# apache/datafusion-comet

Hardware: NVIDIA H100
Metric: rows/sec on TPC-H Q1 filter+agg (higher is better)
Workload: dtype i128

## Files before the change

datafusion-comet_b200/csrc/agg.cpp:

```cpp
#include "exec_internal.h"
#include "../../include/comet_b200.h"

#include "aot_kernels.h"
#include "ranges.h"

#include <algorithm>
#include <mutex>

namespace cb200 {

static std::mutex g_profile_mu;
static std::map<std::string, std::vector<int>> g_range_profile;

void reset_range_profiles() {
    std::lock_guard<std::mutex> lk(g_profile_mu);
    g_range_profile.clear();
}

namespace {

enum class Strategy { Undecided, Dense, Table, Stream };
enum Level { SAFE = 0, TYPE = 1, TIGHT = 2 };
constexpr int DENSE_MAX_GROUPS = 64;

constexpr int GK = CB_GID_RANGES;
struct HashFlags { int w[CB_HFLAG_WORDS]; };
int64_t round_ids(int64_t n) { return (n + GK - 1) / GK * GK; }

using ValueMasks = uint64_t[CB_MAX_COLS * 2];

uint64_t identity_word(int kind) { return kind == W_MIN ? 0x7fffffffffffffffull : kind == W_MAX ? 0x8000000000000000ull : 0; }

std::vector<int> decode_gid(int g, const std::vector<int>& cards) {
    std::vector<int> code(cards.size());
    for (int k = (int)cards.size() - 1; k >= 0; k--) { code[(size_t)k] = g % cards[(size_t)k]; g /= cards[(size_t)k]; }
    return code;
}

int grid_for(const ExecContext* ctx, int n_tiles) { return std::max(1, std::min(ctx->num_sms, n_tiles)); }

struct Kernel {
    PipelineSpec spec;
    GeneratedKernel g;
    std::shared_ptr<CompiledModule> mod;
};

void launch_named(ExecContext* ctx, const Kernel& k, const char* name, dim3 grid, dim3 block, void** args) {
    cuda_check(cudaLaunchKernel((const void*)k.mod->kernel(name), grid, block, args, 0, ctx->stream), name);
    ctx->kernel_launches++;
}

struct DenseState {
    std::vector<int> cards;
    std::vector<bool> has_null;
    DeviceBufP totals, spill, partials;
    int groups = 0;

    void regroup(ExecContext* ctx, int n_words, const std::vector<int>& word_kinds, const std::vector<int>& new_cards) {
        int new_groups = 1;
        for (int c : new_cards) new_groups *= c;
        std::vector<uint64_t> oldt((size_t)groups * n_words * 2), newt((size_t)new_groups * n_words * 2);
        cuda_check(cudaMemcpy(oldt.data(), totals->ptr, oldt.size() * 8, cudaMemcpyDeviceToHost), "regroup D2H");
        for (size_t i = 0; i < (size_t)new_groups * n_words; i++) newt[i * 2] = identity_word(word_kinds[i % (size_t)n_words]);
        for (int g = 0; g < groups; g++) {
            const std::vector<int> code = decode_gid(g, cards);
            int ng = 0, mul = 1;
            for (int k = (int)cards.size() - 1; k >= 0; k--) {
                int cd = code[(size_t)k];
                if (has_null[(size_t)k] && cd == cards[(size_t)k] - 1) cd = new_cards[(size_t)k] - 1;
                ng += cd * mul;
                mul *= new_cards[(size_t)k];
            }
            memcpy(&newt[(size_t)ng * n_words * 2], &oldt[(size_t)g * n_words * 2], (size_t)n_words * 16);
        }
        totals = host_to_device(newt.data(), newt.size() * 8, ctx, "regroup H2D");
        groups = new_groups;
    }

    void finalize(ExecContext* ctx, const Kernel& last, cb::FinParams fp, bool ungrouped, const std::vector<DType>& schema,
                  const std::vector<DictionaryP>& key_dicts, Batch& out) const {
        TraceSpan ts("agg.finalize");
        const GeneratedKernel& g = last.g;
        const int ng = groups;
        fp.totals = (cb::u64*)totals->ptr;
        fp.n_groups = ng;
        std::vector<size_t> off_v, off_n;
        size_t total_bytes = 0;
        auto take = [&](size_t n) { size_t o = total_bytes; total_bytes += (n + 15) / 16 * 16; return o; };
        for (size_t i = 0; i < g.out_cols.size(); i++) { off_v.push_back(take((size_t)ng * g.out_bytes[i])); off_n.push_back(take((size_t)ng)); }
        size_t off_present = take((size_t)ng);
        auto dbuf = std::make_shared<DeviceBuf>(total_bytes);
        for (size_t i = 0; i < g.out_cols.size(); i++) {
            fp.out[i] = (cb::u8*)dbuf->ptr + off_v[i];
            fp.outv[i] = (cb::u8*)dbuf->ptr + off_n[i];
        }
        fp.present = (cb::u8*)dbuf->ptr + off_present;
        void* args[] = {&fp};
        cuda_check(cudaLaunchKernel((const void*)last.mod->kernel(g.finalize_entry), dim3((ng + 127) / 128), dim3(128), args, 0, ctx->stream), "finalize launch");
        ctx->kernel_launches++;
        std::vector<uint8_t> hbuf(total_bytes);
        cuda_check(cudaMemcpyAsync(hbuf.data(), dbuf->ptr, total_bytes, cudaMemcpyDeviceToHost, ctx->stream), "agg results D2H"); ctx->d2h_bytes += (int64_t)(total_bytes);
        ctx->check_device_errors();
        const uint8_t* pres = hbuf.data() + off_present;
        std::vector<int> rows;
        for (int gi = 0; gi < ng; gi++) if (ungrouped || pres[(size_t)gi]) rows.push_back(gi);
        out.n_rows = (int64_t)rows.size();
// ... 166 lines not shown

struct KeyTable {
    DeviceBufP hkeys;
    int64_t hcap = 0;

    void ensure(ExecContext* ctx, const Kernel& k, IdRows& rows, int64_t incoming, int64_t remaining, int64_t rows_scanned, bool merging) {
        cudaStream_t st = ctx->stream;
        rows.ensure_flags(ctx);
        HashFlags hf;
        int64_t cnt[GK];
        const int64_t cur = rows.read_flags(ctx, hf, cnt);
        const int64_t need = cur + incoming;
        if (need + 2 >= INT32_MAX) throw ExecError(16, "", "more than 2^31 groups in one partition; lower spark.comet.b200.chunkRows");
        bool relocated = false;
        if (need > rows.max_groups) {
            int64_t nm = std::max<int64_t>(need, rows.max_groups + rows.max_groups / 4);
            if (remaining > 0 && rows_scanned == 0 && merging) {
                nm = std::max(nm, need + remaining);
            }
            if (remaining > 0 && rows_scanned > 0 && cur > 0) {
                const double ratio = std::min(1.0, 1.3 * (double)cur / (double)rows_scanned);
                const int64_t est = cur + incoming + (int64_t)(ratio * (double)remaining);
                nm = std::max(nm, std::min<int64_t>(est, cur + incoming + remaining));
            }
            if (nm + 2 + GK >= INT32_MAX) nm = INT32_MAX - 3 - GK;
            relocated = cur > 0;
            rows.grow(ctx, k, cnt, round_ids(nm), true);
        }
        int64_t cap = std::max<int64_t>(hcap, 1 << 16);
        while (cap < 2 * std::max(need, rows.max_groups)) cap <<= 1;
        if (cap != hcap || relocated) {
            auto nkeys = cap != hcap ? std::make_shared<DeviceBuf>((size_t)cap * 16) : hkeys;
            cuda_check(cudaMemsetAsync(nkeys->ptr, 0xff, (size_t)cap * 16, st), "memset key slots");
            if (cur > 0) {
                const cb::u64* kog = (const cb::u64*)rows.hkey_of_gid->ptr;
                int rr = (int)(rows.max_groups / GK);
                const int* ctr = (const int*)rows.hflags->ptr + CB_HFLAG_CTR;
                cb::u64* kp = (cb::u64*)nkeys->ptr;
                cb::u32 mask = (cb::u32)(cap - 1);
                void* a2[] = {&kog, &rr, &ctr, &kp, &mask};
                launch_named(ctx, k, "cb_hash_rehash", dim3((unsigned)((rows.max_groups + 255) / 256)), dim3(256), a2);
                cuda_check(cudaStreamSynchronize(st), "rehash");
            }
            hkeys = nkeys; hcap = cap;
        }
    }
};

struct StreamState {
    double ratio = 1.0;
    DeviceBufP reserved_snap;

    void ensure_rows(ExecContext* ctx, const Kernel& k, IdRows& rows, const int64_t cnt[GK], int64_t want_groups) {
        rows.ensure_flags(ctx);
        if (rows.htotals && want_groups <= rows.max_groups) return;
        rows.grow(ctx, k, cnt, round_ids(std::max<int64_t>(want_groups, rows.max_groups + rows.max_groups / 2)), false);
    }
    void snapshot_reserved(ExecContext* ctx, const IdRows& rows, int n_words, bool restore) {
        const size_t bytes = (size_t)2 * n_words * 16;
        if (!reserved_snap || reserved_snap->bytes < bytes) reserved_snap = std::make_shared<DeviceBuf>(bytes);
        cb::u64* tail = (cb::u64*)rows.htotals->ptr + (size_t)rows.max_groups * n_words * 2;
        if (restore) cuda_check(cudaMemcpyAsync(tail, reserved_snap->ptr, bytes, cudaMemcpyDeviceToDevice, ctx->stream), "restore reserved groups");
        else cuda_check(cudaMemcpyAsync(reserved_snap->ptr, tail, bytes, cudaMemcpyDeviceToDevice, ctx->stream), "snapshot reserved groups");
    }
};

struct AggNode : FusedBase {
    std::vector<ExprP> keys;
    std::vector<AggExpr> aggs;
    std::vector<std::vector<int>> state_cols;
    AggMode mode = AggMode::Partial;
    bool reads_rows = true;
    bool all_partial = true;
    std::vector<bool> is_state_col;
    bool ungrouped = false;
    bool emitted = false;
    std::vector<Batch> outq;
    size_t outq_pos = 0;
    std::vector<int> assume_bits;

    std::vector<bool> key_has_null;
    std::vector<bool> col_nullable;
    std::vector<DictionaryP> key_dicts;
    struct DevDict { StringDictDev d; std::vector<DeviceBufP> bufs; int host_known = 0; };
    std::vector<std::shared_ptr<DevDict>> dev_dicts;

    int n_words = 0, key_words = 1;
    std::vector<int> word_kinds, role_words;
    Kernel last;
    bool have_totals() const { return last.mod != nullptr; }

    Strategy strategy = Strategy::Undecided;
    DenseState dense;
    KeyTable table;
    IdRows rows;

    std::vector<int> observed_bits;
    int64_t rows_scanned = 0;
    std::string profile_key;
    DeviceBufP vmask;
    StreamState stream;

    int assume_for(int child_col, Level lv) const {
        const DType& t = child->schema[(size_t)child_col];
        if (!t.is_decimal() || lv == SAFE || !reads_rows || is_state_col[(size_t)child_col]) return 0;
        int k = r_bitlen(r_prec_max(t.precision));
        if ((size_t)child_col < assume_bits.size() && assume_bits[(size_t)child_col] > 0) k = std::min(k, assume_bits[(size_t)child_col]);
        if (lv == TIGHT && !observed_bits.empty() && observed_bits[(size_t)child_col] >= 0) k = std::min(k, observed_bits[(size_t)child_col] + 2);
        return std::min(k, 126);
    }

    PipelineSpec make_spec(const Batch* b, Strategy st, int n_groups, Level lv = TYPE) const {
        const bool hash = st == Strategy::Table || st == Strategy::Stream;
        PipelineSpec s;
        s.cols = stage_cols(b);
        for (auto& c : s.cols) {
            c.assume_bits = assume_for(c.src_index, lv);
            c.layout_nullable = b && col_nullable[(size_t)c.src_index];
        }
        s.predicates = to_slots(predicates, slot_of);
        s.sink = SinkKind::Agg;
        s.mode = mode;
        s.ungrouped = ungrouped;
        s.hash = hash;
        s.keys = to_slots(keys, slot_of);
        for (size_t k = 0; k < keys.size(); k++) s.key_nullable.push_back(b ? key_has_null[k] : false);
        for (auto& a : aggs) {
            AggExpr c = a;
            if (a.mode == AggMode::Partial) {
                c.children = to_slots(a.children, slot_of);
                if (a.filter) c.filter = to_slots({a.filter}, slot_of)[0];
            }
            s.aggs.push_back(c);
        }
        for (auto& sc : state_cols) {
            std::vector<int> v;
            for (int ci : sc) v.push_back(slot_of.at(ci));
            s.state_slots.push_back(v);
        }
        if (hash) {
            s.threads = ctx->hash_threads;
            s.tile = 2 * ctx->hash_threads;
            s.stream = st == Strategy::Stream;
        }
        GeneratedKernel probe = generate_pipeline(s);
        size_t acc = (!ungrouped && !hash) ? (size_t)std::max(n_groups, 1) * probe.n_words * s.threads * 8 : 0;
        while (acc + 2 * (size_t)probe.stage_bytes + 1024 > SMEM_BUDGET && s.threads > 32) {
            s.threads /= 2;
            acc /= 2;
        }
        if (acc + 2 * (size_t)probe.stage_bytes + 1024 > SMEM_BUDGET)
            throw Unsupported(hash ? "too many state / input columns to stage in shared memory for the hash aggregate kernel"
                                   : "too many groups x aggregates for the thread-private accumulators of the dense path");
        s.stages = (int)std::max<size_t>(2, std::min<size_t>(6, (SMEM_BUDGET - 1024 - acc) / (size_t)probe.stage_bytes));
        return s;
    }

    std::vector<PipelineSpec> build_specs() const override {
        bool hash = false;
        for (auto& k : keys) if (!k->type.is_string() && k->type.id != TypeId::Bool) hash = true;
        std::vector<PipelineSpec> out{make_spec(nullptr, hash ? Strategy::Table : Strategy::Dense, ungrouped ? 1 : 6)};
        if (hash && mode == AggMode::Partial && all_partial) out.push_back(make_spec(nullptr, Strategy::Stream, 6));
        return out;
    }

    Kernel compile(const PipelineSpec& spec) {
        Kernel k{spec, generate_pipeline(spec), nullptr};
        k.mod = jit_get(k.g, true);
        if (have_totals() && k.g.key_words != key_words) throw ExecError(15, "", "internal: group key packing changed between launches");
        if (have_totals() && (k.g.n_words != n_words || k.g.word_kinds != word_kinds || k.g.role_words != role_words)) widen(k);
        n_words = k.g.n_words;
        word_kinds = k.g.word_kinds;
        role_words = k.g.role_words;
        key_words = k.g.key_words;
        return k;
    }

    void widen(const Kernel& k) {
        GeneratedKernel from;
        from.n_words = n_words;
        from.word_kinds = word_kinds;
        from.role_words = role_words;
        const std::vector<int> map = widen_word_map(from, k.g);
        if (map.empty()) throw ExecError(15, "", "internal: accumulator layout changed between launches");
        const bool is_dense = strategy == Strategy::Dense;
        DeviceBufP& t = is_dense ? dense.totals : rows.htotals;
        const size_t n_rows = is_dense ? (size_t)dense.groups : (size_t)rows.max_groups + 2;
        auto nt = std::make_shared<DeviceBuf>(n_rows * (size_t)k.g.n_words * 16);
        for (int w = 0; w < k.g.n_words; w++)
            cuda_check(cudaMemcpy2DAsync((char*)nt->ptr + (size_t)w * 16, (size_t)k.g.n_words * 16, (const char*)t->ptr + (size_t)map[(size_t)w] * 16,
                                         (size_t)n_words * 16, 16, n_rows, cudaMemcpyDeviceToDevice, ctx->stream), "widen totals");
        cuda_check(cudaStreamSynchronize(ctx->stream), "widen totals");
        t = nt;
    }

    void clear_vmask() {
        if (!vmask) vmask = std::make_shared<DeviceBuf>(CB_MAX_COLS * 16);
        cuda_check(cudaMemsetAsync(vmask->ptr, 0, CB_MAX_COLS * 16, ctx->stream), "memset vmask");
    }
    void copy_vmask(ValueMasks& masks) {
        cuda_check(cudaMemcpyAsync(masks, vmask->ptr, sizeof(ValueMasks), cudaMemcpyDeviceToHost, ctx->stream), "read value masks"); ctx->d2h_bytes += (int64_t)(sizeof(ValueMasks));
    }
    static std::vector<int> mask_bits(const PipelineSpec& spec, const ValueMasks& masks) {
        std::vector<int> seen(spec.cols.size(), -1);
        for (size_t i = 0; i < spec.cols.size(); i++) {
            if (!spec.cols[i].type.is_decimal()) continue;
            uint64_t lo = masks[2 * i], hi = masks[2 * i + 1];
            seen[i] = hi ? 64 + r_bitlen(hi) : r_bitlen(lo);
        }
        return seen;
    }
    void observe(const std::vector<int>& seen) {
        for (size_t i = 0; i < seen.size(); i++)
            if (seen[i] >= 0) observed_bits[(size_t)used_cols[i]] = std::max(observed_bits[(size_t)used_cols[i]], seen[i]);
    }

    int prepare_key(Batch& b, size_t k) {
        int ci = keys[k]->index;
        Column& c = b.cols[ci];
        if (c.type.id == TypeId::Bool) return 2;
        if (!c.type.is_string()) return -1;
        if (c.is_dict) {
            key_dicts[k] = c.dict;
            return (int)c.dict->values().size();
        }
        if (!dev_dicts[k]) {
            auto dd = std::make_shared<DevDict>();
            const int64_t cap = 1 << 16;
            const int max_codes = 4096;
            const int64_t bytes_cap = 1 << 20;
            auto alloc = [&](size_t n) { auto bfr = std::make_shared<DeviceBuf>(n); cuda_check(cudaMemsetAsync(bfr->ptr, 0, bfr->bytes, ctx->stream), "memset dict"); dd->bufs.push_back(bfr); return bfr->ptr; };
            dd->d.tags = (unsigned long long*)alloc((size_t)cap * 8);
            dd->d.slot_code = (int*)alloc((size_t)cap * 4);
            dd->d.capacity = cap;
            dd->d.n_codes = (int*)alloc(64);
            dd->d.bytes_used = (unsigned long long*)((char*)dd->d.n_codes + 16);
            dd->d.err = (int*)((char*)dd->d.n_codes + 32);
            dd->d.max_codes = max_codes;
            dd->d.code_off = (long long*)alloc((size_t)max_codes * 8);
            dd->d.code_len = (int*)alloc((size_t)max_codes * 4);
            dd->d.bytes = (unsigned char*)alloc((size_t)bytes_cap);
            dd->d.bytes_cap = bytes_cap;
            dev_dicts[k] = dd;
            key_dicts[k] = std::make_shared<Dictionary>();
        }
        DevDict& dd = *dev_dicts[k];
        if (!c.offsets || !c.chars) throw Unsupported("string key column without offsets/chars buffers");
        auto row_slot = std::make_shared<DeviceBuf>((size_t)b.n_rows * 4);
        auto codes = std::make_shared<DeviceBuf>((size_t)b.n_rows * 4);
        launch_dict_encode(dd.d, (const int*)c.offsets->ptr, (const unsigned char*)c.chars->ptr, c.validity ? (const unsigned char*)c.validity->ptr : nullptr,
                           b.n_rows, (int*)row_slot->ptr, (int*)codes->ptr, ctx->stream);
        ctx->kernel_launches += 2;
        int hdr[12];
        cuda_check(cudaMemcpyAsync(hdr, dd.d.n_codes, sizeof(hdr), cudaMemcpyDeviceToHost, ctx->stream), "dict header");
        cuda_check(cudaStreamSynchronize(ctx->stream), "dict encode");
        int n_codes = hdr[0], derr = hdr[8];
        if (derr & CB_DICT_FULL) throw Unsupported("plain Utf8 group key with more distinct values than the device dictionary holds (dictionary-encode the column)");
        if (derr & CB_DICT_COLLISION) throw ExecError(14, "", "64-bit hash collision between distinct group key strings");
        if (n_codes > dd.host_known) {
            std::vector<long long> off((size_t)n_codes);
            std::vector<int> len((size_t)n_codes);
            cuda_check(cudaMemcpy(off.data(), dd.d.code_off, (size_t)n_codes * 8, cudaMemcpyDeviceToHost), "dict offsets");
            cuda_check(cudaMemcpy(len.data(), dd.d.code_len, (size_t)n_codes * 4, cudaMemcpyDeviceToHost), "dict lengths");
            for (int i = dd.host_known; i < n_codes; i++) {
                std::string s((size_t)len[(size_t)i], '\0');
                if (len[(size_t)i]) cuda_check(cudaMemcpy(&s[0], dd.d.bytes + off[(size_t)i], (size_t)len[(size_t)i], cudaMemcpyDeviceToHost), "dict bytes");
                key_dicts[k]->append(s);
            }
            dd.host_known = n_codes;
        }
        c.data = codes;
        c.phys = Phys::I32;
        c.is_dict = true;
        c.dict = key_dicts[k];
        return n_codes;
    }

    void consume(Batch& b) {
        for (int ci : used_cols) if (b.cols[(size_t)ci].validity) col_nullable[(size_t)ci] = true;
        std::vector<int> nc(keys.size());
        std::vector<bool> hn(keys.size());
        for (size_t k = 0; k < keys.size(); k++) {
            int card = prepare_key(b, k);
            const Column& c = b.cols[keys[k]->index];
            hn[k] = key_has_null[k] || c.validity != nullptr;
            nc[k] = card < 0 ? -1 : std::max(card, 1) + (hn[k] ? 1 : 0);
            if (!dense.cards.empty() && nc[k] >= 0) nc[k] = std::max(nc[k], dense.cards[k]);
        }
        bool densifiable = true;
        for (int c : nc) if (c < 0) densifiable = false;
        int n_groups = 1;
        if (densifiable) for (int c : nc) { n_groups *= c; if (n_groups > 1 << 20) break; }
        const bool needs_hash = !ungrouped && (!densifiable || n_groups > DENSE_MAX_GROUPS);
        key_has_null = hn;
        if (observed_bits.empty()) observed_bits.assign(child->schema.size(), -1);
        if (strategy == Strategy::Undecided || (strategy == Strategy::Dense && needs_hash)) {
            if (strategy == Strategy::Dense) {
                leave_dense();
                ctx->agg_strategies |= CB200_AGG_MIGRATED;
            }
            strategy = !needs_hash ? Strategy::Dense : sample_stream(b) ? Strategy::Stream : Strategy::Table;
            ctx->agg_strategies |= strategy == Strategy::Dense ? CB200_AGG_DENSE : strategy == Strategy::Stream ? CB200_AGG_STREAM : CB200_AGG_TABLE;
        }
        if (strategy == Strategy::Dense) consume_dense(b, nc, n_groups);
        else if (strategy == Strategy::Table) consume_table(b);
        else consume_stream(b);
    }

    void consume_dense(Batch& b, const std::vector<int>& nc, int n_groups) {
        if (have_totals() && nc != dense.cards) {
            if (n_words == 0) throw ExecError(15, "", "internal: regroup before layout");
            dense.regroup(ctx, n_words, word_kinds, nc);
        }
        dense.cards = nc;
        dense.has_null = key_has_null;
        const int64_t SAMPLE = 1 << 20;
        bool have_obs = false;
        for (int ci : used_cols) if (child->schema[(size_t)ci].is_decimal() && observed_bits[(size_t)ci] >= 0) have_obs = true;
        if (reads_rows && !have_obs && b.n_rows > 2 * SAMPLE) {
            profile_key = pipeline_signature(make_spec(&b, Strategy::Dense, n_groups, SAFE));
            std::lock_guard<std::mutex> lk(g_profile_mu);
            auto it = g_range_profile.find(profile_key);
            if (it != g_range_profile.end() && it->second.size() == observed_bits.size()) {
                observed_bits = it->second;
                for (int ci : used_cols) if (child->schema[(size_t)ci].is_decimal() && observed_bits[(size_t)ci] >= 0) have_obs = true;
            }
        }
        if (!reads_rows) {
            run_range(b, 0, b.n_rows, n_groups, SAFE);
        } else if (!have_obs && b.n_rows > 2 * SAMPLE) {
            run_range(b, 0, SAMPLE, n_groups, TYPE);
            run_range(b, SAMPLE, b.n_rows, n_groups, TIGHT);
        } else {
            run_range(b, 0, b.n_rows, n_groups, have_obs ? TIGHT : TYPE);
        }
        if (!profile_key.empty()) {
            std::lock_guard<std::mutex> lk(g_profile_mu);
            if (g_range_profile.size() > 256) g_range_profile.clear();
            g_range_profile[profile_key] = observed_bits;
        }
    }

    void leave_dense() {
        if (mode == AggMode::Final) throw Unsupported("group cardinality grew past the dense path mid-stream in a Final aggregate");
        if (have_totals()) {
            Batch early;
            dense.finalize(ctx, last, certified_params(), ungrouped, schema, key_dicts, early);
            if (early.n_rows > 0) outq.push_back(std::move(early));
        }
        last = Kernel();
        dense = DenseState();
        n_words = 0; word_kinds.clear(); role_words.clear(); rows_scanned = 0;
    }

    void run_range(Batch& b, int64_t row0, int64_t row1, int n_groups, Level lv) {
        TraceSpan tsr("agg.run_range");
        while (true) {
            Kernel k;
            {
                TraceSpan ts("agg.codegen+jit");
                k = compile(make_spec(&b, Strategy::Dense, n_groups, lv));
            }
            const int64_t max_rows = (int64_t)ctx->num_sms * k.g.threads * (1ll << CB_RPT_LOG2) / 1024 * 1024;
            int64_t r0 = row0;
            while (r0 < row1 && launch_one(b, r0, std::min(row1, r0 + max_rows), n_groups, k, lv)) r0 += max_rows;
            if (r0 >= row1) return;
            if (lv == SAFE) throw ExecError(15, "", "internal: value-mask validation failed without assumptions");
            lv = lv == TIGHT ? TYPE : SAFE;
            row0 = r0;
        }
    }

    bool launch_one(Batch& b, int64_t r0, int64_t r1, int n_groups, const Kernel& k, Level lv) {
        cudaStream_t st = ctx->stream;
        size_t tot_bytes = (size_t)n_groups * n_words * 16;
        if (!have_totals()) {
            dense.totals = std::make_shared<DeviceBuf>(tot_bytes);
            dense.groups = n_groups;
        }
        if (!dense.spill || dense.spill->bytes < tot_bytes) {
            dense.spill = std::make_shared<DeviceBuf>(tot_bytes);
            cuda_check(cudaMemsetAsync(dense.spill->ptr, 0, dense.spill->bytes, st), "memset spill");
        }
        clear_vmask();
        cb::PipeParams p;
        fill_inputs(p, b, k.g.tile, r0, r1);
        bind_str_masks(p, k.spec, b);
        int grid = grid_for(ctx, p.n_tiles);
        size_t part_bytes = (size_t)grid * tot_bytes;
        if (!dense.partials || dense.partials->bytes < part_bytes) dense.partials = std::make_shared<DeviceBuf>(part_bytes);
        p.n_groups = n_groups;
        for (size_t i = 0; i < dense.cards.size() && i < CB_MAX_KEYS; i++) p.key_card[i] = dense.cards[i];
        p.partials = (cb::u8*)dense.partials->ptr;
        p.spill = (cb::u64*)dense.spill->ptr;
        p.vmask = (cb::u64*)vmask->ptr;
        launch(k.mod->kernel(k.g.entry), dim3(grid), dim3(k.g.threads + 32), k.g.dyn_smem(n_groups), &p);
        ctx->pipeline_rows += r1 - r0;
        ValueMasks masks;
        copy_vmask(masks);
        const int errs = ctx->take_device_errors();
        const std::vector<int> seen = mask_bits(k.spec, masks);
        bool ok = true;
        for (size_t i = 0; i < seen.size(); i++)
            if (k.spec.cols[i].assume_bits > 0 && seen[i] > k.spec.cols[i].assume_bits) ok = false;
        observe(seen);
        if (!ok) {
            cuda_check(cudaMemsetAsync(dense.spill->ptr, 0, dense.spill->bytes, st), "memset spill");
            ctx->agg_range_reruns++;
            return false;
        }
        ctx->raise_device_errors(errs);
        ctx->agg_range_levels |= lv == TIGHT ? CB200_RANGE_TIGHT : lv == TYPE ? CB200_RANGE_TYPE : CB200_RANGE_SAFE;
        rows_scanned += r1 - r0;
        cb::FinParams fp;
        memset(&fp, 0, sizeof(fp));
        fp.partials = (const cb::u64*)dense.partials->ptr;
        fp.spill = (cb::u64*)dense.spill->ptr;
        fp.totals = (cb::u64*)dense.totals->ptr;
        fp.n_ctas = grid;
        fp.n_groups = n_groups;
        fp.first = have_totals() ? 0 : 1;
        fp.err = ctx->d_err;
        int total_words = n_groups * n_words;
        void* args[] = {&fp};
        cuda_check(cudaLaunchKernel((const void*)k.mod->kernel("cb_fold"), dim3((total_words + 127) / 128), dim3(128), args, 0, st), "fold launch");
        ctx->kernel_launches++;
        last = k;
        return true;
    }

    void launch_id_rows(Batch& b, int64_t r0, int64_t r1, const Kernel& k, bool with_table) {
        clear_vmask();
        cb::PipeParams p;
        fill_inputs(p, b, k.g.tile, r0, r1);
        bind_str_masks(p, k.spec, b);
        p.hkeys = with_table ? (cb::u64*)table.hkeys->ptr : nullptr;
        p.hkey_of_gid = (cb::u64*)rows.hkey_of_gid->ptr;
        p.htotals = (cb::u64*)rows.htotals->ptr;
        p.hmask = with_table ? (cb::u32)(table.hcap - 1) : 0;
        p.max_groups = (cb::i32)rows.max_groups;
        p.hflags = (cb::i32*)rows.hflags->ptr;
        p.vmask = (cb::u64*)vmask->ptr;
        p.n_groups = 2;
        launch(k.mod->kernel(k.g.entry), dim3(grid_for(ctx, p.n_tiles)), dim3(k.g.threads + 32), k.g.dyn_smem(0), &p);
    }

    void consume_table(Batch& b) {
        const Kernel k = compile(make_spec(&b, Strategy::Table, 2, SAFE));
        {
            TraceSpan ts("hash.ensure_table");
            table.ensure(ctx, k, rows, b.n_rows, child->rows_hint(), rows_scanned, mode != AggMode::Partial || !all_partial);
        }
        launch_id_rows(b, 0, b.n_rows, k, true);
        ctx->pipeline_rows += b.n_rows;
        ValueMasks masks;
        int flags[8];
        copy_vmask(masks);
        cuda_check(cudaMemcpyAsync(flags, rows.hflags->ptr, sizeof(flags), cudaMemcpyDeviceToHost, ctx->stream), "read hash flags"); ctx->d2h_bytes += (int64_t)(sizeof(flags));
        ctx->check_device_errors();
        if (flags[0] & CB_HF_FULL) throw ExecError(15, "", "internal: hash table full");
        if (flags[0] & CB_HF_WIDE_KEY) throw Unsupported("decimal(p > 18) group key whose value does not fit 64 bits");
        observe(mask_bits(k.spec, masks));
        rows_scanned += b.n_rows;
        last = k;
    }

    int64_t stream_launch(Batch& b, int64_t r0, int64_t r1, const Kernel& k, HashFlags& hf, int64_t cnt[GK]) {
        launch_id_rows(b, r0, r1, k, false);
        ValueMasks masks;
        copy_vmask(masks);
        ctx->check_device_errors();
        const int64_t total = rows.read_flags(ctx, hf, cnt);
        if (hf.w[0] & CB_HF_WIDE_KEY) throw Unsupported("decimal(p > 18) group key whose value does not fit 64 bits");
        if (!(hf.w[0] & CB_HF_FULL)) observe(mask_bits(k.spec, masks));
        return total;
    }
    bool sample_stream(Batch& b) {
        if (mode != AggMode::Partial || !all_partial || ctx->stream_agg_min_rows < 0) return false;
        if (b.n_rows + std::max<int64_t>(child->rows_hint(), 0) < ctx->stream_agg_min_rows || b.n_rows == 0) return false;
        const Kernel k = compile(make_spec(&b, Strategy::Stream, 2, SAFE));
        const int64_t sample = std::min<int64_t>(b.n_rows, 1 << 20);
        HashFlags hf;
        int64_t cnt[GK] = {0};
        stream.ensure_rows(ctx, k, rows, cnt, 2 * sample + 4096);
        const int64_t runs = stream_launch(b, 0, sample, k, hf, cnt);
        stream.ratio = (hf.w[0] & CB_HF_FULL) ? 1.0 : (double)runs / (double)sample;
        memset(&hf, 0, sizeof(hf));
        rows.write_flags(ctx, hf);
        IdRows::init_totals(ctx, k, (cb::u64*)rows.htotals->ptr, rows.max_groups, 2);
        if (stream.ratio <= ctx->stream_agg_max_ratio) return true;
        rows = IdRows();
        n_words = 0; word_kinds.clear(); role_words.clear();
        return false;
    }
    void consume_stream(Batch& b) {
        const Kernel k = compile(make_spec(&b, Strategy::Stream, 2, SAFE));
        HashFlags before, hf;
        int64_t cnt0[GK], cnt[GK];
        const int64_t cur = rows.read_flags(ctx, before, cnt0);
        const int64_t remaining = std::max<int64_t>(child->rows_hint(), 0);
        int64_t want = cur + std::min<int64_t>(b.n_rows, (int64_t)(1.25 * stream.ratio * (double)b.n_rows) + 65536);
        if (!rows.htotals || want > rows.max_groups) want += std::min<int64_t>(remaining, (int64_t)(1.25 * stream.ratio * (double)remaining));
        int64_t handed_out;
        while (true) {
            {
                TraceSpan ts("stream.ensure_rows");
                stream.ensure_rows(ctx, k, rows, cnt0, want);
            }
            stream.snapshot_reserved(ctx, rows, n_words, false);
            handed_out = stream_launch(b, 0, b.n_rows, k, hf, cnt);
            if (!(hf.w[0] & CB_HF_FULL)) break;
            ctx->agg_stream_reruns++;
            stream.snapshot_reserved(ctx, rows, n_words, true);
            for (int r = 0; r < GK; r++) before.w[CB_HFLAG_CTR + r] = (int)cnt0[r];
            rows.write_flags(ctx, before);
            want = cur + b.n_rows + GK;
        }
        ctx->pipeline_rows += b.n_rows;
        if (b.n_rows > 0) stream.ratio = std::max(stream.ratio, (double)(handed_out - cur) / (double)b.n_rows);
        rows_scanned += b.n_rows;
        last = k;
    }

    u128r certificate(size_t ai) const {
        const AggExpr& a = aggs[ai];
        if (!(a.kind == AggKind::Sum || a.kind == AggKind::Avg) || !a.datatype.is_decimal()) return 0;
        std::vector<u128r> bounds(child->schema.size(), RSAT);
        for (size_t c = 0; c < bounds.size(); c++)
            if (child->schema[c].is_decimal() && !observed_bits.empty())
                bounds[c] = observed_bits[c] < 0 ? 0 : (observed_bits[c] >= 127 ? RSAT : (u128r)1 << observed_bits[c]);
        if (a.mode == AggMode::Partial) return expr_maxabs(*a.children[0], bounds);
        return bounds[(size_t)state_cols[ai][0]];
    }
    cb::FinParams certified_params() const {
        cb::FinParams fp;
        memset(&fp, 0, sizeof(fp));
        fp.err = ctx->d_err;
        for (size_t ai = 0; ai < aggs.size() && ai < CB_MAX_OUT; ai++) {
            const u128r b = certificate(ai);
            fp.cert_b[ai][0] = b >= RSAT ? ~0ull : (uint64_t)b;
            fp.cert_b[ai][1] = b >= RSAT ? ~0ull : (uint64_t)(b >> 64);
            const bool direct = aggs[ai].mode != AggMode::Partial || aggs[ai].children[0]->kind == ExprKind::Bound;
            if (b < RSAT && b != 0 && direct) fp.cert_b[ai][1] |= 1ull << 63;
        }
        return fp;
    }

    bool next(Batch& out) override {
        if (!emitted) aggregate_input();
        if (outq_pos >= outq.size()) return false;
        out = std::move(outq[outq_pos++]);
        return true;
    }
    void aggregate_input() {
        if (keys.size() > CB_MAX_KEYS) throw Unsupported("more than 4 group keys");
        key_has_null.assign(keys.size(), false);
        col_nullable.assign(child->schema.size(), false);
        key_dicts.assign(keys.size(), nullptr);
        dev_dicts.assign(keys.size(), nullptr);
        Batch in;
        while (child->next(in)) {
            if (in.n_rows == 0) continue;
            consume(in);
            ctx->check_device_errors();
        }
        emitted = true;
        if (!have_totals()) {
            if (!ungrouped) return;
            last = compile(make_spec(nullptr, Strategy::Dense, 1));
            std::vector<uint64_t> id((size_t)n_words * 2, 0);
            for (int w = 0; w < n_words; w++) id[(size_t)w * 2] = identity_word(word_kinds[(size_t)w]);
            dense.totals = std::make_shared<DeviceBuf>(id.size() * 8);
            cuda_check(cudaMemcpyAsync(dense.totals->ptr, id.data(), id.size() * 8, cudaMemcpyHostToDevice, ctx->stream), "identity totals");
            cuda_check(cudaStreamSynchronize(ctx->stream), "identity totals sync");
            dense.groups = 1;
        }
        Batch result;
        if (strategy == Strategy::Table || strategy == Strategy::Stream) rows.finalize(ctx, last, certified_params(), key_dicts, result);
        else dense.finalize(ctx, last, certified_params(), ungrouped, schema, key_dicts, result);
        outq.push_back(std::move(result));
    }
};

}

ExecNodeP make_agg_node(const OperatorP& agg_op, const ExecNodeP& src, const std::vector<ExprP>& preds, const std::vector<ExprP>& cols, ExecContext* ctx,
                        const std::vector<int>& assume_bits) {
    auto n = std::make_shared<AggNode>();
    n->ctx = ctx;
    n->child = src;
    n->schema = agg_op->schema;
    n->predicates = preds;
    n->mode = agg_op->mode;
    n->ungrouped = agg_op->grouping.empty();
    n->assume_bits = assume_bits;
    std::vector<ExprP> roots = preds;
    for (auto& gexp : agg_op->grouping) {
        ExprP k = substitute(gexp, cols);
        if (k->kind != ExprKind::Bound) throw Unsupported("computed group keys (only plain column keys are fused)");
        n->keys.push_back(k);
        roots.push_back(k);
    }
    n->is_state_col.assign(src->schema.size(), false);
    n->reads_rows = agg_op->mode == AggMode::Partial;
    for (auto& a : agg_op->aggs) {
        AggExpr c = a;
        std::vector<int> sc;
        if (a.mode == AggMode::Partial) {
            n->reads_rows = true;
            for (auto& ch : c.children) { ch = substitute(ch, cols); roots.push_back(ch); }
            if (c.filter) { c.filter = substitute(c.filter, cols); roots.push_back(c.filter); }
        } else {
            n->all_partial = false;
            for (size_t k = 0; k < agg_state_types(a).size(); k++) {
                ExprP e = cols.at((size_t)a.state_at + k);
                if (e->kind != ExprKind::Bound) throw Unsupported("final aggregate over computed state columns");
                sc.push_back(e->index);
                n->is_state_col[(size_t)e->index] = true;
                roots.push_back(e);
            }
        }
        n->state_cols.push_back(sc);
        n->aggs.push_back(c);
    }
    n->assign_slots(roots);
    if (n->used_cols.empty()) {
        int best = -1, best_w = 1 << 30;
        for (size_t c = 0; c < src->schema.size(); c++) {
            const DType& t = src->schema[c];
            if (t.is_string()) continue;
            int w = std::max(1, phys_bytes(phys_of(t)));
            if (w < best_w) { best = (int)c; best_w = w; }
        }
        if (best < 0) throw Unsupported("COUNT(*) over a child with only string columns");
        n->used_cols.push_back(best);
        n->slot_of[best] = 0;
    }
    return n;
}

}
```

datafusion-comet_b200/csrc/exec.cpp:

```cpp
#include "exec_internal.h"

#include <cstdlib>
#include <ctime>
#include <mutex>

namespace cb200 {

enum { ERR_I128_OVERFLOW = 0, ERR_ANSI_OVERFLOW = 1, ERR_ORDER_DEPENDENT = 2, ERR_DIVIDE_BY_ZERO = 3, ERR_ARROW_DIVIDE_BY_ZERO = 4, ERR_DICT_CODE = 5,
       ERR_WIDE_MINMAX = 6 };

bool trace_on() {
    static int on = -1;
    if (on < 0) { const char* e = getenv("CB200_TRACE"); on = (e && *e && *e != '0') ? 1 : 0; }
    return on == 1;
}
double now_ms() {
    struct timespec ts;
    clock_gettime(CLOCK_MONOTONIC, &ts);
    return ts.tv_sec * 1e3 + ts.tv_nsec * 1e-6;
}
TraceSpan::TraceSpan(const char* n) : name(n), t0(trace_on() ? now_ms() : 0) {}
TraceSpan::~TraceSpan() {
    if (trace_on()) { static const double tz = now_ms(); const double t1 = now_ms(); fprintf(stderr, "[cb200 trace] %-28s %8.3f ms   (ends at +%.3f ms)\n", name, t1 - t0, t1 - tz); }
}
// ... 326 lines not shown
        return cudaMemcpyAsync(dst, src, n, cudaMemcpyHostToDevice, ctx->stream);
    }

    void upload(std::vector<ArrowArray>& arrs, int64_t total, Batch& out) {
        TraceSpan ts("source.upload");
        out.n_rows = total;
        out.cols.clear();
        out.cols.resize(schema.size());
        cudaStream_t st = ctx->stream;
        for (size_t c = 0; c < schema.size(); c++) {
            Column& col = out.cols[c];
            col.type = schema[c];
            bool any_nulls = false;
            for (auto& a : arrs) {
                ArrowArray* ch = a.children[c];
                if (ch->null_count != 0 && ch->buffers[0]) any_nulls = true;
            }
            if (any_nulls) {
                col.validity = std::make_shared<DeviceBuf>((size_t)(total + 7) / 8 + 8);
                cuda_check(cudaMemsetAsync(col.validity->ptr, 0, col.validity->bytes, st), "memset validity");
            }
            std::vector<DeviceBufP> temps;
            if (col_is_dict[c]) {
                col.is_dict = true;
                col.dict = dicts[c];
                int w = dict_index_width[c];
                bool need_remap = false;
                std::vector<std::vector<int32_t>> remaps;
                for (auto& a : arrs) {
                    remaps.push_back(unify_dict(c, a.children[c]->dictionary));
                    if (!remaps.back().empty()) need_remap = true;
                }
                if (!need_remap) {
                    col.phys = w == 1 ? Phys::I8 : w == 2 ? Phys::I16 : Phys::I32;
                    col.data = std::make_shared<DeviceBuf>((size_t)total * w);
                } else {
                    col.phys = Phys::I32;
                    col.data = std::make_shared<DeviceBuf>((size_t)total * 4);
                }
                int64_t row = 0;
                for (size_t k = 0; k < arrs.size(); k++) {
                    ArrowArray* ch = arrs[k].children[c];
                    const char* src = (const char*)ch->buffers[1] + ch->offset * w;
                    if (!need_remap) {
                        cuda_check(h2d((char*)col.data->ptr + row * w, src, (size_t)ch->length * w), "H2D dict codes");
                    } else {
                        auto tmp = std::make_shared<DeviceBuf>((size_t)ch->length * w);
                        temps.push_back(tmp);
                        cuda_check(h2d(tmp->ptr, src, (size_t)ch->length * w), "H2D dict codes");
                        std::vector<int32_t> table = remaps[k];
                        if (table.empty()) { table.resize((size_t)ch->dictionary->length); for (size_t i = 0; i < table.size(); i++) table[i] = (int32_t)i; }
                        DeviceBufP dt = host_to_device(table.data(), table.size() * 4, ctx, "H2D remap table");
                        ctx->h2d_bytes += (int64_t)(table.size() * 4);
                        temps.push_back(dt);
                        launch_remap_codes(tmp->ptr, w, ch->length, (const int*)dt->ptr, (int)table.size(), (int*)col.data->ptr + row, st);
                    }
                    row += ch->length;
                }
            } else if (schema[c].is_string()) {
                int64_t total_chars = 0;
                for (auto& a : arrs) {
                    ArrowArray* ch = a.children[c];
                    const int32_t* off = (const int32_t*)ch->buffers[1] + ch->offset;
                    total_chars += off[ch->length] - off[0];
                }
                if (total_chars > INT32_MAX) throw Unsupported("more than 2 GiB of string data in one chunk");
                col.chars = std::make_shared<DeviceBuf>((size_t)total_chars + 16);
                std::vector<int32_t> offs((size_t)total + 1);
                int64_t row = 0;
                int32_t base = 0;
                for (auto& a : arrs) {
                    ArrowArray* ch = a.children[c];
                    const int32_t* off = (const int32_t*)ch->buffers[1] + ch->offset;
                    for (int64_t i = 0; i < ch->length; i++) offs[(size_t)(row + i)] = base + (off[i] - off[0]);
                    int32_t nchars = off[ch->length] - off[0];
                    if (nchars) cuda_check(h2d((char*)col.chars->ptr + base, (const char*)ch->buffers[2] + off[0], (size_t)nchars), "H2D chars");
                    base += nchars;
                    row += ch->length;
                }
                offs[(size_t)total] = base;
                col.offsets = host_to_device(offs.data(), offs.size() * 4, ctx, "H2D offsets");
                ctx->h2d_bytes += (int64_t)(offs.size() * 4);
                col.phys = Phys::I32;
            } else {
                col.phys = phys_of(schema[c]);
                int w = schema[c].arrow_width();
                if (w == 0) {
                    col.data = std::make_shared<DeviceBuf>((size_t)(total + 7) / 8 + 8);
                    cuda_check(cudaMemsetAsync(col.data->ptr, 0, col.data->bytes, st), "memset bool");
                    int64_t row = 0;
                    for (auto& a : arrs) {
                        ArrowArray* ch = a.children[c];
                        append_bits((uint32_t*)col.data->ptr, row, (const uint8_t*)ch->buffers[1], ch->offset, ch->length, temps);
                        row += ch->length;
                    }
                } else {
                    col.data = std::make_shared<DeviceBuf>((size_t)total * w);
                    int64_t row = 0;
                    for (auto& a : arrs) {
                        ArrowArray* ch = a.children[c];
                        cuda_check(h2d((char*)col.data->ptr + row * w, (const char*)ch->buffers[1] + ch->offset * w, (size_t)ch->length * w), "H2D column");
                        row += ch->length;
                    }
                }
            }
            if (any_nulls) {
                int64_t row = 0, nulls = 0;
                for (auto& a : arrs) {
                    ArrowArray* ch = a.children[c];
                    bool has = ch->null_count != 0 && ch->buffers[0];
                    append_bits((uint32_t*)col.validity->ptr, row, has ? (const uint8_t*)ch->buffers[0] : nullptr, ch->offset, ch->length, temps);
                    nulls += has ? (ch->null_count < 0 ? 1 : ch->null_count) : 0;
                    row += ch->length;
                }
                col.null_count = nulls;
            }
            if (!temps.empty()) cuda_check(cudaStreamSynchronize(st), "temp buffers");
        }
    }

    void append_bits(uint32_t* dst, int64_t row, const uint8_t* src, int64_t src_off, int64_t n, std::vector<DeviceBufP>& temps) {
        if (n <= 0) return;
        if (src && (row & 7) == 0 && (src_off & 7) == 0 && ((n & 7) == 0)) {
            cuda_check(h2d((char*)dst + (row >> 3), src + (src_off >> 3), (size_t)(n >> 3)), "H2D bitmap");
            return;
        }
        const uint8_t* dsrc = nullptr;
        int64_t doff = 0;
        if (src) {
            int64_t b0 = src_off >> 3, b1 = (src_off + n + 7) >> 3;
            auto tmp = std::make_shared<DeviceBuf>((size_t)(b1 - b0) + 8);
            temps.push_back(tmp);
            cuda_check(h2d(tmp->ptr, src + b0, (size_t)(b1 - b0)), "H2D bitmap");
            dsrc = (const uint8_t*)tmp->ptr;
            doff = src_off & 7;
        }
        launch_bitmap_append(dst, row, dsrc, doff, n, ctx->stream);
    }
};

struct TableSource : ExecNode {
    std::shared_ptr<DeviceTable> table;
    ExecContext* ctx = nullptr;
    bool done = false;
    TableSource(std::shared_ptr<DeviceTable> t, const std::vector<DType>& fields, ExecContext* c) : table(std::move(t)), ctx(c) {
        schema = fields;
        if (table->cols.size() != fields.size()) throw PlanError("bound device table has " + std::to_string(table->cols.size()) + " columns, scan declares " + std::to_string(fields.size()));
    }
    int64_t pos = 0;
    bool packed = false;
    int64_t rows_hint() const override { return table->n_rows - pos; }
    bool next(Batch& out) override {
        if (done) return false;
        if (table->needs_packing && !packed) {
            for (auto& c : table->cols) {
                if (c.valid_bytes && !c.validity) c.validity = bytes_to_bitmap(c.valid_bytes, table->n_rows, ctx);
                if (c.bool_bytes && !c.data) c.data = bytes_to_bitmap(c.bool_bytes, table->n_rows, ctx);
            }
            packed = true;
        }
        const int64_t chunk = std::max<int64_t>(1024, ctx->chunk_rows / 1024 * 1024);
        const int64_t r0 = pos, r1 = std::min(table->n_rows, pos + chunk);
        pos = r1;
        if (pos >= table->n_rows) done = true;
        out.n_rows = r1 - r0;
        out.cols = table->cols;
// ... 433 lines not shown
```

datafusion-comet_b200/csrc/exec.h:

```cpp
#pragma once
#include "arrow_abi.h"
#include "codegen.h"
#include "jit.h"
#include "plan.h"

#include <cuda_runtime.h>
#include <climits>
#include <memory>
#include <string>
#include <unordered_map>
#include <vector>

namespace cb200 {

struct ExecError : std::runtime_error {
    int code;
    std::string error_class;
    ExecError(int c, const std::string& cls, const std::string& msg) : std::runtime_error(msg), code(c), error_class(cls) {}
};

void cuda_check(cudaError_t e, const char* what);

struct TraceSpan {
    const char* name;
    double t0;
    explicit TraceSpan(const char* n);
    ~TraceSpan();
};
bool trace_on();
double now_ms();
void set_alloc_stream(cudaStream_t s);
size_t release_cached_device_memory();
void reset_range_profiles();

struct DeviceBuf {
    void* ptr = nullptr;
    size_t bytes = 0;
    bool owned = true;
    cudaStream_t stream = nullptr;
    std::shared_ptr<void> owner;
    DeviceBuf() {}
    DeviceBuf(size_t n);
    DeviceBuf(void* p, size_t n) : ptr(p), bytes(n), owned(false) {}
    ~DeviceBuf();
    DeviceBuf(const DeviceBuf&) = delete;
    DeviceBuf& operator=(const DeviceBuf&) = delete;
};
using DeviceBufP = std::shared_ptr<DeviceBuf>;

class Dictionary {
  public:
    const std::vector<std::string>& values() const { return values_; }
    int32_t intern(std::string v) {
        auto it = index_.find(v);
        if (it != index_.end()) return it->second;
        if (values_.size() >= (size_t)INT32_MAX) throw Unsupported("more than 2^31 distinct strings in one dictionary");
        const int32_t code = (int32_t)values_.size();
        index_.emplace(v, code);
        values_.push_back(std::move(v));
        return code;
    }
    void append(std::string v) {
        index_.emplace(v, (int32_t)values_.size());
        values_.push_back(std::move(v));
    }
    int32_t find(const std::string& v) const {
        auto it = index_.find(v);
        return it == index_.end() ? -1 : it->second;
    }

  private:
    std::vector<std::string> values_;
    std::unordered_map<std::string, int32_t> index_;
};
using DictionaryP = std::shared_ptr<Dictionary>;

struct Column {
    DType type;
    Phys phys = Phys::I32;
    bool is_dict = false;
    DictionaryP dict;
    DeviceBufP data, validity;
    DeviceBufP offsets, chars;
    DeviceBufP valid_bytes;
    DeviceBufP bool_bytes;
    int64_t null_count = 0;
    bool on_host = false;
    std::vector<uint8_t> h_data;
    std::vector<uint8_t> h_valid;
    std::vector<int32_t> h_offsets;
};

struct Batch {
    int64_t n_rows = 0;
    std::vector<Column> cols;
};

struct ExecContext {
    int device = 0;
    cudaStream_t stream = nullptr;
    int num_sms = 132;
    int64_t chunk_rows = 1ll << 26;
    int hash_threads = 512;
    int64_t stream_agg_min_rows = 4 << 20;
    double stream_agg_max_ratio = 0.5;
    int batch_size = 8192;
    int* d_err = nullptr;
    int* h_err = nullptr;
    int64_t kernel_launches = 0;
    cudaEvent_t ev0 = nullptr, ev1 = nullptr;
    bool ev_pending = false;
    double pipeline_ms = 0;
    int64_t pipeline_launches = 0;
    int64_t pipeline_rows = 0;
    int64_t h2d_bytes = 0, d2h_bytes = 0;
    int64_t scan_pruned_row_groups = 0, scan_pruned_rows = 0;
    int64_t scan_pruned_pages = 0, scan_page_pruned_rows = 0;
    int64_t agg_strategies = 0;
    int64_t agg_range_levels = 0;
    int64_t agg_range_reruns = 0;
    int64_t sort_rows = 0, sort_passes = 0, sort_pass_rows = 0;
    int64_t sort_select_rows = 0;
    int64_t join_build_rows = 0, join_probe_rows = 0, join_out_rows = 0;
    int64_t join_cond_pairs = 0;
    double partition_ids_ms = 0, partition_place_ms = 0, partition_gather_ms = 0;
    int64_t agg_table_grows = 0;
    int64_t agg_stream_reruns = 0;
    std::vector<int64_t> partition_starts;
    void check_device_errors() { raise_device_errors(take_device_errors()); }
    int take_device_errors();
    void raise_device_errors(int e);
    void collect_timing();
};

struct ExecNode {
    std::vector<DType> schema;
    virtual ~ExecNode() {}
    virtual bool next(Batch& out) = 0;
    virtual std::vector<std::shared_ptr<ExecNode>> children() const { return {}; }
    virtual std::vector<PipelineSpec> build_specs() const { return {}; }
    virtual void push_filters(const std::vector<ExprP>&) {}
    virtual int64_t rows_hint() const { return -1; }
};
using ExecNodeP = std::shared_ptr<ExecNode>;

struct DeviceTable {
    int64_t n_rows = 0;
    std::vector<Column> cols;
    bool needs_packing = false;
};

struct PlanInputs {
    std::vector<ArrowArrayStream*> streams;
    std::vector<std::shared_ptr<DeviceTable>> tables;
};
ExecNodeP build_exec(const OperatorP& op, ExecContext* ctx, PlanInputs* inputs);

ExecNodeP make_native_scan(const OperatorP& op, ExecContext* ctx);

bool to_arrow_layout(Batch& b, ExecContext* ctx);
void export_batch(Batch& b, ExecContext* ctx, ArrowArray* out_arrays, ArrowSchema* out_schemas, int n_cols, int64_t row0, int64_t n_rows);

void register_memory_file(const std::string& name, const uint8_t* p, size_t n);
std::string describe_parquet(const std::string& path);

std::vector<GeneratedKernel> plan_kernels_for_build(const OperatorP& op, const std::vector<int>& assume_bits = {});

}
```

Measured before the change: 38.35 billion.

## Batch dense-agg range launches with a single mask readback and intern small string keys on host

Dense aggregation no longer launches, syncs and reads back value masks once per row range. It now enqueues every range kernel with its own partials, spill and mask slots, does one D2H copy and one sync, then validates and folds each range. Small plain-Utf8 key columns are interned on the host and only the codes are uploaded, and device dictionary codes are remapped to a shared host dictionary. The cost is more device memory for per-range partials, and wasted work when a range fails validation and later ranges must rerun.

```diff
diff --git a/datafusion-comet_b200/csrc/agg.cpp b/datafusion-comet_b200/csrc/agg.cpp
--- a/datafusion-comet_b200/csrc/agg.cpp
+++ b/datafusion-comet_b200/csrc/agg.cpp
@@ -22,6 +22,9 @@
 enum class Strategy { Undecided, Dense, Table, Stream };
 enum Level { SAFE = 0, TYPE = 1, TIGHT = 2 };
 constexpr int DENSE_MAX_GROUPS = 64;
+constexpr int KEY_DICT_MAX_CODES = 4096;
+constexpr int64_t KEY_DICT_MAX_BYTES = 1 << 20;
+const char* const KEY_DICT_FULL = "plain Utf8 group key with more distinct values than the device dictionary holds (dictionary-encode the column)";
 
 constexpr int GK = CB_GID_RANGES;
 struct HashFlags { int w[CB_HFLAG_WORDS]; };
@@ -354,8 +357,10 @@
     std::vector<bool> key_has_null;
     std::vector<bool> col_nullable;
     std::vector<DictionaryP> key_dicts;
-    struct DevDict { StringDictDev d; std::vector<DeviceBufP> bufs; int host_known = 0; };
+    struct DevDict { StringDictDev d; std::vector<DeviceBufP> bufs; int host_known = 0; std::vector<int32_t> to_key; };
     std::vector<std::shared_ptr<DevDict>> dev_dicts;
+    std::vector<int64_t> key_dict_bytes;
+    std::vector<std::vector<int32_t>> host_codes;
 
     int n_words = 0, key_words = 1;
     std::vector<int> word_kinds, role_words;
@@ -372,6 +377,11 @@
     std::string profile_key;
     DeviceBufP vmask;
     StreamState stream;
+    DeviceBufP range_slots;
+    std::vector<std::pair<cudaEvent_t, cudaEvent_t>> range_events;
+    ~AggNode() override {
+        for (auto& e : range_events) { cudaEventDestroy(e.first); if (e.second) cudaEventDestroy(e.second); }
+    }
 
     int assume_for(int child_col, Level lv) const {
         const DType& t = child->schema[(size_t)child_col];
@@ -496,11 +506,13 @@
             key_dicts[k] = c.dict;
             return (int)c.dict->values().size();
         }
+        if (!key_dicts[k]) key_dicts[k] = std::make_shared<Dictionary>();
+        if (!c.h_offsets.empty()) return intern_on_host(c, b.n_rows, k);
         if (!dev_dicts[k]) {
             auto dd = std::make_shared<DevDict>();
             const int64_t cap = 1 << 16;
-            const int max_codes = 4096;
-            const int64_t bytes_cap = 1 << 20;
+            const int max_codes = KEY_DICT_MAX_CODES;
+            const int64_t bytes_cap = KEY_DICT_MAX_BYTES;
             auto alloc = [&](size_t n) { auto bfr = std::make_shared<DeviceBuf>(n); cuda_check(cudaMemsetAsync(bfr->ptr, 0, bfr->bytes, ctx->stream), "memset dict"); dd->bufs.push_back(bfr); return bfr->ptr; };
             dd->d.tags = (unsigned long long*)alloc((size_t)cap * 8);
             dd->d.slot_code = (int*)alloc((size_t)cap * 4);
@@ -514,7 +526,6 @@
             dd->d.bytes = (unsigned char*)alloc((size_t)bytes_cap);
             dd->d.bytes_cap = bytes_cap;
             dev_dicts[k] = dd;
-            key_dicts[k] = std::make_shared<Dictionary>();
         }
         DevDict& dd = *dev_dicts[k];
         if (!c.offsets || !c.chars) throw Unsupported("string key column without offsets/chars buffers");
@@ -527,7 +538,7 @@
         cuda_check(cudaMemcpyAsync(hdr, dd.d.n_codes, sizeof(hdr), cudaMemcpyDeviceToHost, ctx->stream), "dict header");
         cuda_check(cudaStreamSynchronize(ctx->stream), "dict encode");
         int n_codes = hdr[0], derr = hdr[8];
-        if (derr & CB_DICT_FULL) throw Unsupported("plain Utf8 group key with more distinct values than the device dictionary holds (dictionary-encode the column)");
+        if (derr & CB_DICT_FULL) throw Unsupported(KEY_DICT_FULL);
         if (derr & CB_DICT_COLLISION) throw ExecError(14, "", "64-bit hash collision between distinct group key strings");
         if (n_codes > dd.host_known) {
             std::vector<long long> off((size_t)n_codes);
@@ -537,15 +548,50 @@
             for (int i = dd.host_known; i < n_codes; i++) {
                 std::string s((size_t)len[(size_t)i], '\0');
                 if (len[(size_t)i]) cuda_check(cudaMemcpy(&s[0], dd.d.bytes + off[(size_t)i], (size_t)len[(size_t)i], cudaMemcpyDeviceToHost), "dict bytes");
-                key_dicts[k]->append(s);
+                dd.to_key.push_back(intern_key(k, std::move(s)));
             }
             dd.host_known = n_codes;
+        }
+        bool identity = true;
+        for (size_t i = 0; i < dd.to_key.size(); i++) identity &= dd.to_key[i] == (int32_t)i;
+        if (!identity) {
+            DeviceBufP table = host_to_device(dd.to_key.data(), dd.to_key.size() * 4, ctx, "H2D key recode table");
+            launch_remap_codes(codes->ptr, 4, b.n_rows, (const int*)table->ptr, (int)dd.to_key.size(), (int*)codes->ptr, ctx->stream);
+            ctx->kernel_launches++;
+            cuda_check(cudaStreamSynchronize(ctx->stream), "key recode");
         }
         c.data = codes;
         c.phys = Phys::I32;
         c.is_dict = true;
         c.dict = key_dicts[k];
-        return n_codes;
+        return (int)key_dicts[k]->values().size();
+    }
+
+    int32_t intern_key(size_t k, std::string v) {
+        Dictionary& d = *key_dicts[k];
+        const size_t before = d.values().size(), len = v.size();
+        const int32_t code = d.intern(std::move(v));
+        if (d.values().size() > before) {
+            key_dict_bytes[k] += (int64_t)len;
+            if (d.values().size() > (size_t)KEY_DICT_MAX_CODES || key_dict_bytes[k] > KEY_DICT_MAX_BYTES) throw Unsupported(KEY_DICT_FULL);
+        }
+        return code;
+    }
+    int intern_on_host(Column& c, int64_t n_rows, size_t k) {
+        std::vector<int32_t>& codes = host_codes[k];
+        codes.assign((size_t)n_rows, 0);
+        const char* chars = (const char*)c.h_data.data();
+        for (int64_t r = 0; r < n_rows; r++) {
+            if (!c.h_valid.empty() && !c.h_valid[(size_t)r]) continue;
+            codes[(size_t)r] = intern_key(k, std::string(chars + c.h_offsets[(size_t)r], (size_t)(c.h_offsets[(size_t)r + 1] - c.h_offsets[(size_t)r])));
+        }
+        c.data = std::make_shared<DeviceBuf>((size_t)n_rows * 4);
+        cuda_check(cudaMemcpyAsync(c.data->ptr, codes.data(), codes.size() * 4, cudaMemcpyHostToDevice, ctx->stream), "H2D key codes");
+        ctx->h2d_bytes += (int64_t)(codes.size() * 4);
+        c.phys = Phys::I32;
+        c.is_dict = true;
+        c.dict = key_dicts[k];
+        return (int)key_dicts[k]->values().size();
     }
 
     void consume(Batch& b) {
@@ -634,8 +680,7 @@
                 k = compile(make_spec(&b, Strategy::Dense, n_groups, lv));
             }
             const int64_t max_rows = (int64_t)ctx->num_sms * k.g.threads * (1ll << CB_RPT_LOG2) / 1024 * 1024;
-            int64_t r0 = row0;
-            while (r0 < row1 && launch_one(b, r0, std::min(row1, r0 + max_rows), n_groups, k, lv)) r0 += max_rows;
+            const int64_t r0 = launch_range(b, row0, row1, max_rows, n_groups, k, lv);
             if (r0 >= row1) return;
             if (lv == SAFE) throw ExecError(15, "", "internal: value-mask validation failed without assumptions");
             lv = lv == TIGHT ? TYPE : SAFE;
@@ -643,62 +688,94 @@
         }
     }
 
-    bool launch_one(Batch& b, int64_t r0, int64_t r1, int n_groups, const Kernel& k, Level lv) {
+    int64_t launch_range(Batch& b, int64_t row0, int64_t row1, int64_t max_rows, int n_groups, const Kernel& k, Level lv) {
         cudaStream_t st = ctx->stream;
-        size_t tot_bytes = (size_t)n_groups * n_words * 16;
+        const int n = (int)((row1 - row0 + max_rows - 1) / max_rows);
+        const size_t tot_bytes = (size_t)n_groups * n_words * 16, part_bytes = (size_t)ctx->num_sms * tot_bytes;
+        const size_t mask_words = CB_MAX_COLS * 2, slots_bytes = (size_t)n * (mask_words * 8 + 4);
         if (!have_totals()) {
             dense.totals = std::make_shared<DeviceBuf>(tot_bytes);
             dense.groups = n_groups;
         }
-        if (!dense.spill || dense.spill->bytes < tot_bytes) {
-            dense.spill = std::make_shared<DeviceBuf>(tot_bytes);
+        if (!dense.spill || dense.spill->bytes < n * tot_bytes) {
+            dense.spill = std::make_shared<DeviceBuf>(n * tot_bytes);
             cuda_check(cudaMemsetAsync(dense.spill->ptr, 0, dense.spill->bytes, st), "memset spill");
         }
-        clear_vmask();
-        cb::PipeParams p;
-        fill_inputs(p, b, k.g.tile, r0, r1);
-        bind_str_masks(p, k.spec, b);
-        int grid = grid_for(ctx, p.n_tiles);
-        size_t part_bytes = (size_t)grid * tot_bytes;
-        if (!dense.partials || dense.partials->bytes < part_bytes) dense.partials = std::make_shared<DeviceBuf>(part_bytes);
-        p.n_groups = n_groups;
-        for (size_t i = 0; i < dense.cards.size() && i < CB_MAX_KEYS; i++) p.key_card[i] = dense.cards[i];
-        p.partials = (cb::u8*)dense.partials->ptr;
-        p.spill = (cb::u64*)dense.spill->ptr;
-        p.vmask = (cb::u64*)vmask->ptr;
-        launch(k.mod->kernel(k.g.entry), dim3(grid), dim3(k.g.threads + 32), k.g.dyn_smem(n_groups), &p);
-        ctx->pipeline_rows += r1 - r0;
-        ValueMasks masks;
-        copy_vmask(masks);
-        const int errs = ctx->take_device_errors();
-        const std::vector<int> seen = mask_bits(k.spec, masks);
-        bool ok = true;
-        for (size_t i = 0; i < seen.size(); i++)
-            if (k.spec.cols[i].assume_bits > 0 && seen[i] > k.spec.cols[i].assume_bits) ok = false;
-        observe(seen);
-        if (!ok) {
-            cuda_check(cudaMemsetAsync(dense.spill->ptr, 0, dense.spill->bytes, st), "memset spill");
-            ctx->agg_range_reruns++;
-            return false;
-        }
-        ctx->raise_device_errors(errs);
-        ctx->agg_range_levels |= lv == TIGHT ? CB200_RANGE_TIGHT : lv == TYPE ? CB200_RANGE_TYPE : CB200_RANGE_SAFE;
-        rows_scanned += r1 - r0;
-        cb::FinParams fp;
-        memset(&fp, 0, sizeof(fp));
-        fp.partials = (const cb::u64*)dense.partials->ptr;
-        fp.spill = (cb::u64*)dense.spill->ptr;
-        fp.totals = (cb::u64*)dense.totals->ptr;
-        fp.n_ctas = grid;
-        fp.n_groups = n_groups;
-        fp.first = have_totals() ? 0 : 1;
-        fp.err = ctx->d_err;
-        int total_words = n_groups * n_words;
-        void* args[] = {&fp};
-        cuda_check(cudaLaunchKernel((const void*)k.mod->kernel("cb_fold"), dim3((total_words + 127) / 128), dim3(128), args, 0, st), "fold launch");
-        ctx->kernel_launches++;
-        last = k;
-        return true;
+        if (!dense.partials || dense.partials->bytes < n * part_bytes) dense.partials = std::make_shared<DeviceBuf>(n * part_bytes);
+        if (!range_slots || range_slots->bytes < slots_bytes) range_slots = std::make_shared<DeviceBuf>(slots_bytes);
+        cuda_check(cudaMemsetAsync(range_slots->ptr, 0, slots_bytes, st), "memset value masks");
+        while ((int)range_events.size() < n) {
+            std::pair<cudaEvent_t, cudaEvent_t> e{nullptr, nullptr};
+            cuda_check(cudaEventCreate(&e.first), "cudaEventCreate");
+            range_events.push_back(e);
+            cuda_check(cudaEventCreate(&range_events.back().second), "cudaEventCreate");
+        }
+        uint64_t* masks_d = (uint64_t*)range_slots->ptr;
+        int* errs_d = (int*)(masks_d + (size_t)n * mask_words);
+        const cudaKernel_t kern = k.mod->kernel(k.g.entry);
+        const size_t smem = k.g.dyn_smem(n_groups);
+        cuda_check(cudaFuncSetAttribute((const void*)kern, cudaFuncAttributeMaxDynamicSharedMemorySize, (int)smem), "cudaFuncSetAttribute(smem)");
+        if (ctx->ev_pending) { cuda_check(cudaStreamSynchronize(st), "stream sync"); ctx->collect_timing(); }
+        std::vector<int> grids((size_t)n);
+        for (int i = 0; i < n; i++) {
+            const int64_t r0 = row0 + i * max_rows, r1 = std::min(row1, r0 + max_rows);
+            cb::PipeParams p;
+            fill_inputs(p, b, k.g.tile, r0, r1);
+            bind_str_masks(p, k.spec, b);
+            grids[(size_t)i] = grid_for(ctx, p.n_tiles);
+            p.n_groups = n_groups;
+            for (size_t j = 0; j < dense.cards.size() && j < CB_MAX_KEYS; j++) p.key_card[j] = dense.cards[j];
+            p.partials = (cb::u8*)dense.partials->ptr + i * part_bytes;
+            p.spill = (cb::u64*)((char*)dense.spill->ptr + i * tot_bytes);
+            p.vmask = (cb::u64*)(masks_d + (size_t)i * mask_words);
+            p.err = errs_d + i;
+            void* args[] = {&p};
+            cuda_check(cudaEventRecord(range_events[(size_t)i].first, st), "event record");
+            cuda_check(cudaLaunchKernel((const void*)kern, dim3(grids[(size_t)i]), dim3(k.g.threads + 32), args, smem, st), "kernel launch");
+            cuda_check(cudaEventRecord(range_events[(size_t)i].second, st), "event record");
+            ctx->kernel_launches++;
+            ctx->pipeline_rows += r1 - r0;
+        }
+        std::vector<uint64_t> slots(slots_bytes / 8 + 1);
+        cuda_check(cudaMemcpyAsync(slots.data(), range_slots->ptr, slots_bytes, cudaMemcpyDeviceToHost, st), "read value masks");
+        ctx->d2h_bytes += (int64_t)slots_bytes;
+        cuda_check(cudaStreamSynchronize(st), "range launches");
+        for (int i = 0; i < n; i++) {
+            float ms = 0;
+            if (cudaEventElapsedTime(&ms, range_events[(size_t)i].first, range_events[(size_t)i].second) == cudaSuccess) { ctx->pipeline_ms += ms; ctx->pipeline_launches++; }
+        }
+        const int* errs = (const int*)(slots.data() + (size_t)n * mask_words);
+        for (int i = 0; i < n; i++) {
+            const int64_t r0 = row0 + i * max_rows, r1 = std::min(row1, r0 + max_rows);
+            const std::vector<int> seen = mask_bits(k.spec, *reinterpret_cast<const ValueMasks*>(slots.data() + (size_t)i * mask_words));
+            bool ok = true;
+            for (size_t j = 0; j < seen.size(); j++)
+                if (k.spec.cols[j].assume_bits > 0 && seen[j] > k.spec.cols[j].assume_bits) ok = false;
+            observe(seen);
+            if (!ok) {
+                cuda_check(cudaMemsetAsync((char*)dense.spill->ptr + i * tot_bytes, 0, (size_t)(n - i) * tot_bytes, st), "memset spill");
+                ctx->agg_range_reruns++;
+                return r0;
+            }
+            ctx->raise_device_errors(errs[i]);
+            ctx->agg_range_levels |= lv == TIGHT ? CB200_RANGE_TIGHT : lv == TYPE ? CB200_RANGE_TYPE : CB200_RANGE_SAFE;
+            rows_scanned += r1 - r0;
+            cb::FinParams fp;
+            memset(&fp, 0, sizeof(fp));
+            fp.partials = (const cb::u64*)((char*)dense.partials->ptr + i * part_bytes);
+            fp.spill = (cb::u64*)((char*)dense.spill->ptr + i * tot_bytes);
+            fp.totals = (cb::u64*)dense.totals->ptr;
+            fp.n_ctas = grids[(size_t)i];
+            fp.n_groups = n_groups;
+            fp.first = have_totals() ? 0 : 1;
+            fp.err = ctx->d_err;
+            int total_words = n_groups * n_words;
+            void* args[] = {&fp};
+            cuda_check(cudaLaunchKernel((const void*)k.mod->kernel("cb_fold"), dim3((total_words + 127) / 128), dim3(128), args, 0, st), "fold launch");
+            ctx->kernel_launches++;
+            last = k;
+        }
+        return row1;
     }
 
     void launch_id_rows(Batch& b, int64_t r0, int64_t r1, const Kernel& k, bool with_table) {
@@ -830,6 +907,8 @@
         col_nullable.assign(child->schema.size(), false);
         key_dicts.assign(keys.size(), nullptr);
         dev_dicts.assign(keys.size(), nullptr);
+        key_dict_bytes.assign(keys.size(), 0);
+        host_codes.assign(keys.size(), {});
         Batch in;
         while (child->next(in)) {
             if (in.n_rows == 0) continue;
diff --git a/datafusion-comet_b200/csrc/exec.cpp b/datafusion-comet_b200/csrc/exec.cpp
--- a/datafusion-comet_b200/csrc/exec.cpp
+++ b/datafusion-comet_b200/csrc/exec.cpp
@@ -432,6 +432,21 @@
                 col.offsets = host_to_device(offs.data(), offs.size() * 4, ctx, "H2D offsets");
                 ctx->h2d_bytes += (int64_t)(offs.size() * 4);
                 col.phys = Phys::I32;
+                if (total <= HOST_UTF8_ROWS) {
+                    col.h_offsets = std::move(offs);
+                    for (auto& a : arrs) {
+                        ArrowArray* ch = a.children[c];
+                        const int32_t* off = (const int32_t*)ch->buffers[1] + ch->offset;
+                        const uint8_t* chars = (const uint8_t*)ch->buffers[2];
+                        col.h_data.insert(col.h_data.end(), chars + off[0], chars + off[ch->length]);
+                        if (!any_nulls) continue;
+                        const uint8_t* vb = ch->null_count != 0 ? (const uint8_t*)ch->buffers[0] : nullptr;
+                        for (int64_t i = 0; i < ch->length; i++) {
+                            const int64_t bit = ch->offset + i;
+                            col.h_valid.push_back(!vb || ((vb[bit >> 3] >> (bit & 7)) & 1) ? 1 : 0);
+                        }
+                    }
+                }
             } else {
                 col.phys = phys_of(schema[c]);
                 int w = schema[c].arrow_width();
diff --git a/datafusion-comet_b200/csrc/exec.h b/datafusion-comet_b200/csrc/exec.h
--- a/datafusion-comet_b200/csrc/exec.h
+++ b/datafusion-comet_b200/csrc/exec.h
@@ -90,6 +90,7 @@
     std::vector<uint8_t> h_valid;
     std::vector<int32_t> h_offsets;
 };
+constexpr int64_t HOST_UTF8_ROWS = 4096;
 
 struct Batch {
     int64_t n_rows = 0;
```

Measured after the change: 39.27 billion (median of 6 runs). 2.4% higher.
